# alpc91/SGRL

Measured on AMD Instinct MI355X. Metric: env-steps/sec (whole node) + SET-actor fwd us/step, 3d_walker mix @8192 envs/GPU, higher is better.
Workload: dtype f64 (dynamics) / f32 (SET actor, obs); 1 GPU; 3D_Walker++ 8 variants x 1024 envs per GPU (config 3), random U(-1,1) actions, auto-reset, SET actor forward on every step, random-init weights; envs_per_gpu=8192, obs_max_len=287, action_max_len=21, replay_gather=none (single rank)

## Files before the change

### include/sgrl_set.h

```cpp
#ifndef SGRL_SET_H
#define SGRL_SET_H

#include <stdint.h>

#ifdef __cplusplus
extern "C" {
#endif

typedef struct sgrl_set sgrl_set;

enum {
  SGRL_SET_EMB0 = 0, SGRL_SET_EMB1, SGRL_SET_EMB2, SGRL_SET_REL_W, SGRL_SET_REL_B, SGRL_SET_FNORM_W, SGRL_SET_FNORM_B,
  SGRL_SET_GENC, SGRL_SET_ENC_W, SGRL_SET_ENC_B, SGRL_SET_GGPROJ, SGRL_SET_L1G_W, SGRL_SET_L1G_B, SGRL_SET_L2G_W,
  SGRL_SET_L2G_B, SGRL_SET_L1NG_W, SGRL_SET_L1NG_B, SGRL_SET_L2NG_W, SGRL_SET_L2NG_B, SGRL_SET_DECG, SGRL_SET_L1M_W,
  SGRL_SET_L1M_B, SGRL_SET_L2M_W, SGRL_SET_L2M_B, SGRL_SET_GPROJ,
  SGRL_SET_NGLOBAL
};
enum {
  SGRL_SET_A_GPROJ = 0, SGRL_SET_A_LG1_W, SGRL_SET_A_LG1_B, SGRL_SET_A_LG2_W, SGRL_SET_A_LG2_B, SGRL_SET_QKV_W,
  SGRL_SET_QKV_B, SGRL_SET_VG_W, SGRL_SET_NGOUT_W, SGRL_SET_NGOUT_B, SGRL_SET_GOUT_W, SGRL_SET_F_GPROJ2,
  SGRL_SET_F_GPROJ3, SGRL_SET_F_LG1_W, SGRL_SET_F_LG1_B, SGRL_SET_F_LG2_W, SGRL_SET_F_LG2_B, SGRL_SET_L3_W,
  SGRL_SET_L3_B, SGRL_SET_L4_W, SGRL_SET_L4_B, SGRL_SET_L5_W, SGRL_SET_L1_W, SGRL_SET_L1_B, SGRL_SET_L2_W,
  SGRL_SET_L2_B, SGRL_SET_N1_W, SGRL_SET_N1_B, SGRL_SET_N2_W, SGRL_SET_N2_B, SGRL_SET_A_GD,
  SGRL_SET_NLAYER
// ... 13 lines not shown
  const void* src0;
  const void* src1;
  int32_t n;
  int32_t kind;
  int32_t a, b;
  float scale;
  int32_t lda, ldb;
  int32_t reserved;
} sgrl_pack_seg;
#define SGRL_SET_NSITES 7
#define SGRL_SET_NEXTRA 2
int sgrl_set_bind_params(sgrl_set* s, const sgrl_pack_seg* segs, int n_segs, const int64_t* offsets, int n_offsets,
                         int64_t total_floats);

int sgrl_set_hold_weights(sgrl_set* s, int hold);

int sgrl_set_graph(sgrl_set* s, int n_morph, const int32_t* morph_L, const int32_t* morph_count, const int32_t* trav,
                   const float* rel);
#define SGRL_SET_GRAPH_CACHE 128

int sgrl_set_forward(sgrl_set* s, const float* obs, int obs_ld, float* act, int act_ld, float max_action, void* stream);

int sgrl_set_forward_q(sgrl_set* s, const float* obs, int obs_ld, const float* action, int action_ld, float* q, int q_ld,
                       void* stream);

int sgrl_set_num_nodes(const sgrl_set* s);
int64_t sgrl_set_workspace_bytes(const sgrl_set* s);
int64_t sgrl_set_generation(const sgrl_set* s);
int sgrl_set_time_forward(sgrl_set* s, const float* obs, int obs_ld, float* act, int act_ld, float max_action,
                          int reps, void* stream, float* ms_out);
int sgrl_set_peek(sgrl_set* s, int which, float* host, int64_t n_floats);
int sgrl_set_debug_stop_after(sgrl_set* s, int stage);
int sgrl_set_debug_small_nodes(sgrl_set* s, int nodes);
int sgrl_set_last_split(const sgrl_set* s);
#define SGRL_SET_FORM_F16X3 2
#define SGRL_SET_FORM_BF16X6 3
int sgrl_set_gemm_form(sgrl_set* s, int form);
int sgrl_set_debug_product(sgrl_set* s, int kind, int form, const float* A, int lda, const float* W, int ldw, const float* bias,
                           float* C, int ldc, int M, int N, int K, const float* rowdiv, const float* aux_in, float* aux_out,
                           void* stream);
int sgrl_set_debug_chain(sgrl_set* s, int kind, const float* A, int lda, int K, const float* Wp, const float* W1, const float* b1, int hid,
                         const float* W2, const float* b2, float* C, int ldc, int M, const float* rowdiv, const float* ln, float* zc,
                         float* z2, float* fn, void* stream);
long long sgrl_set_debug_redos(int reset);
const char* sgrl_set_last_error(void);

#ifdef __cplusplus
}
#endif
#endif
```

### sgrl_amd/csrc/set_actor.hip

```cpp
#include <hip/hip_runtime.h>

#include <algorithm>
#include <cmath>
#include <cstdint>
#include <cstdlib>
#include <cstring>
#include <string>
#include <type_traits>
#include <vector>

#include "../../include/sgrl.h"
#include "../../include/sgrl_set.h"
#include "../../include/sgrl_train.h"
#include "gemm_f32.h"
#include "chain_f16.h"
#include "stream_pick.h"

namespace {

thread_local std::string g_set_err;
int sfail(int code, const std::string& msg) { g_set_err = msg; return code; }
#define SHIP_TRY(expr)                                                                     \
  do {                                                                                     \
    hipError_t _e = (expr);                                                                \
// ... 156 lines not shown
      }
      case SGRL_PACK_SUBMAT: {
        const int r = i / sg.b, c = i % sg.b;
        v = s0[(size_t)r * sg.lda + c];
        break;
      }
      default: break;
    }
    w[sg.dst + i] = v;
  }
}

__global__ void k_relbias(const float* rel, const float* Wr, const float* br, float* relb, const int32_t* m_off,
                          const int32_t* m_L, int n_morph) {
  const int k = blockIdx.x;
  if (k >= n_morph) return;
  const int L = m_L[k], off = m_off[k];
  for (int i = threadIdx.x; i < 2 * L * L; i += blockDim.x) {
    const int h = i / (L * L), ij = i % (L * L);
    const float* r = rel + (size_t)(off / 2) * 3 + ij * 3;
    relb[off + i] = Wr[h * 3] * r[0] + Wr[h * 3 + 1] * r[1] + Wr[h * 3 + 2] * r[2] + br[h];
  }
}

struct EnvTab {
  const int32_t* env_off;
  const int32_t* env_L;
  const int32_t* env_relb;
};
__global__ __launch_bounds__(256) void k_attention(const float* __restrict__ qkv, const float* __restrict__ U,
                                                   const float* __restrict__ gdir, const float* relb, EnvTab et,
                                                   int use_bias, const float* __restrict__ b_ng, const float* __restrict__ GD,
                                                   float* delta_dbg, float* g1, float* ng, int ng_ld,
                                                   const float* __restrict__ ln_w, const float* __restrict__ ln_b) {
  constexpr int LMAX = 14;
  __shared__ float sc[2 * LMAX * LMAX];
  __shared__ float gd[2 * LMAX * 3 * 2];
  __shared__ float dl[LMAX][128];
  const int e = blockIdx.x, t = threadIdx.x;
  const int n0 = et.env_off[e], L = et.env_L[e];
  {
    const int sub = t & 7;
    for (int idx = t >> 3; idx < 2 * L * L; idx += 32) {
      const int h = idx / (L * L), i = (idx / L) % L, j = idx % L;
      const float4* q = reinterpret_cast<const float4*>(qkv + (size_t)(n0 + i) * 768 + h * 128);
      const float4* k = reinterpret_cast<const float4*>(qkv + (size_t)(n0 + j) * 768 + 256 + h * 128);
      float s = 0.f;
#pragma unroll
      for (int u = 0; u < 4; u++) {
        const float4 a = q[sub + 8 * u], b = k[sub + 8 * u];
        s += a.x * b.x + a.y * b.y + a.z * b.z + a.w * b.w;
      }
      s += __shfl_xor(s, 1, 64); s += __shfl_xor(s, 2, 64); s += __shfl_xor(s, 4, 64);
      if (sub == 0) sc[idx] = use_bias ? s + relb[et.env_relb[e] + idx] : s;
    }
  }
  __syncthreads();
  if (t < 2 * L) {
    float* row = sc + t * L;
    float mx = row[0];
    for (int j = 1; j < L; j++) mx = fmaxf(mx, row[j]);
    float sum = 0.f;
    for (int j = 0; j < L; j++) { row[j] = expf(row[j] - mx); sum += row[j]; }
    for (int j = 0; j < L; j++) row[j] = row[j] / sum;
  }
  __syncthreads();
  for (int idx = t; idx < 2 * L * 6; idx += 256) {
    const int h = idx / (L * 6), i = (idx / 6) % L, se = idx % 6;
// ... 63 lines not shown
      for (int i = 0; i < LT; i++)
        if (i0 + i < L) {
          float4 o = out[i];
          const float px = __shfl_xor(o.x, 32, 64), py = __shfl_xor(o.y, 32, 64), pz = __shfl_xor(o.z, 32, 64), pw = __shfl_xor(o.w, 32, 64);
          o = h == 0 ? make_float4(o.x + px, o.y + py, o.z + pz, o.w + pw) : make_float4(px + o.x, py + o.y, pz + o.z, pw + o.w);
          if ((i & 1) == h) {
            if (quantity != 0) {
              *reinterpret_cast<float4*>(g1 + ((size_t)(n0 + i0 + i) * 3 + (quantity - 1)) * 128 + c4) = o;
            } else {
              o.x += bb.x; o.y += bb.y; o.z += bb.z; o.w += bb.w;
              *reinterpret_cast<float4*>(&dl[i0 + i][c4]) = o;
              if (delta_dbg) *reinterpret_cast<float4*>(delta_dbg + (size_t)(n0 + i0 + i) * 128 + c4) = o;
            }
          }
        }
    };
    for (int i0 = 0; i0 < L; i0 += 4) body(std::integral_constant<int, 4>{}, i0);
  }
  __syncthreads();
  const int lane = t & 63;
  const float w0 = ln_w[lane], w1 = ln_w[64 + lane], b0 = ln_b[lane], b1 = ln_b[64 + lane];
  for (int i = t >> 6; i < L; i += 4) {
    float* row = ng + (size_t)(n0 + i) * ng_ld;
    const float v0 = row[lane] + dl[i][lane], v1 = row[64 + lane] + dl[i][64 + lane];
    const float mu = wave_sum_f32(v0 + v1) * (1.f / 128.f);
    const float d0 = v0 - mu, d1 = v1 - mu;
    const float var = wave_sum_f32(d0 * d0 + d1 * d1) * (1.f / 128.f);
    const float inv = 1.0f / sqrtf(var + 1e-5f);
    row[lane] = d0 * inv * w0 + b0;
    row[64 + lane] = d1 * inv * w1 + b1;
  }
}

__global__ __launch_bounds__(256) void k_add_ln(const float* x, int ldx, const float* delta, int ldd, const float* w,
                                                const float* b, float* out1, int ld1, float* out2, int ld2, int N) {
  const int row = blockIdx.x * 4 + (threadIdx.x >> 6), lane = threadIdx.x & 63;
  if (row >= N) return;
  float v0 = x[(size_t)row * ldx + lane], v1 = x[(size_t)row * ldx + 64 + lane];
  if (delta) { v0 += delta[(size_t)row * ldd + lane]; v1 += delta[(size_t)row * ldd + 64 + lane]; }
  const float mu = wave_sum_f32(v0 + v1) * (1.f / 128.f);
  const float d0 = v0 - mu, d1 = v1 - mu;
  const float var = wave_sum_f32(d0 * d0 + d1 * d1) * (1.f / 128.f);
  const float inv = 1.0f / sqrtf(var + 1e-5f);
  const float y0 = d0 * inv * w[lane] + b[lane], y1 = d1 * inv * w[64 + lane] + b[64 + lane];
  if (out1) { out1[(size_t)row * ld1 + lane] = y0; out1[(size_t)row * ld1 + 64 + lane] = y1; }
  if (out2) { out2[(size_t)row * ld2 + lane] = y0; out2[(size_t)row * ld2 + 64 + lane] = y1; }
}

__global__ __launch_bounds__(128) void k_equiv(const float* __restrict__ T, const float* __restrict__ W5,
                                               const float* __restrict__ g1, float* g, float* outg, int N) {
  __shared__ float Ts[8 * 96];
  const int t = threadIdx.x, n0 = blockIdx.x * 8;
  const int rows = min(8, N - n0) * 3;
  for (int o = t; o < 8 * 96; o += 128) Ts[o] = (n0 + o / 96 < N) ? T[(size_t)n0 * 96 + o] : 0.f;
  float w[32];
#pragma unroll
  for (int c = 0; c < 32; c++) w[c] = W5[t * 32 + c];
  __syncthreads();
#pragma unroll
  for (int rb = 0; rb < 24; rb += 8) {
    if (rb >= rows) break;
    float gv[8], g1v[8];
#pragma unroll
    for (int r = 0; r < 8; r++) {
      const size_t row = (size_t)n0 * 3 + (rb + r < rows ? rb + r : 0);
      gv[r] = g[row * D + t];
// ... 44 lines not shown
  if (n >= N) return;
  float vec[3];
  const float mq = m2[(size_t)n * 32 + c];
  for (int s = 0; s < 3; s++) {
    float v = z[(size_t)n * 96 + s * 32 + c] * mq;
    for (int off = 16; off > 0; off >>= 1) v += __shfl_xor(v, off, 32);
    vec[s] = v;
  }
  if (c < 3) {
    const int env = nt.node_env[n], limb = nt.node_limb[n];
    const float* o = obs + (size_t)env * obs_ld + 41 * limb + 3 * (5 + c);
    const float a = o[0] * vec[0] + o[1] * vec[1] + o[2] * vec[2];
    act[(size_t)env * act_ld + 3 * limb + c] = max_action * tanhf(a);
  }
}

__global__ __launch_bounds__(256) void k_q_head(const float* __restrict__ c, const float* __restrict__ w, const float* __restrict__ b,
                                                const float* __restrict__ fn, NodeTab nt, float* q, int q_ld, int N) {
  const int n = blockIdx.x * 4 + (threadIdx.x >> 6), lane = threadIdx.x & 63;
  if (n >= N) return;
  const float* row = c + (size_t)n * 256;
  float v = row[lane] * w[lane] + row[64 + lane] * w[64 + lane] + row[128 + lane] * w[128 + lane] + row[192 + lane] * w[192 + lane];
  v = wave_sum_f32(v);
  if (lane == 0) q[(size_t)nt.node_env[n] * q_ld + nt.node_limb[n]] = (v + b[0]) / fn[n];
}

}

struct GraphCfg {
  std::vector<int32_t> key_i;
  std::vector<float> key_f;
  int n_env = 0, N = 0, n_morph = 0, TM = 0, Lmax = 0;
  int split_env = 0, split_node = 0;
  int32_t *d_node_env = nullptr, *d_node_limb = nullptr, *d_node_mnode = nullptr, *d_trav = nullptr;
  int32_t *d_env_off = nullptr, *d_env_L = nullptr, *d_env_relb = nullptr, *d_m_off = nullptr, *d_m_L = nullptr;
  float *d_rel = nullptr, *d_relb = nullptr;
  uint64_t last_use = 0;
  void release() {
    void* ptrs[] = {d_node_env, d_node_limb, d_node_mnode, d_trav, d_env_off, d_env_L, d_env_relb, d_m_off, d_m_L, d_rel, d_relb};
    for (void* q : ptrs) if (q) (void)hipFree(q);
  }
};

struct sgrl_set {
  const float* w = nullptr;
  int64_t off[SGRL_SET_NW];
  bool have_w = false, have_graph = false;
  int n_env = 0, N = 0, n_morph = 0, TM = 0, Lmax = 0;
  int split_env = 0, split_node = 0;
  int last_split = 0;
  int32_t *d_node_env = nullptr, *d_node_limb = nullptr, *d_node_mnode = nullptr, *d_trav = nullptr;
  int32_t *d_env_off = nullptr, *d_env_L = nullptr, *d_env_relb = nullptr, *d_m_off = nullptr, *d_m_L = nullptr;
  float *d_rel = nullptr, *d_relb = nullptr;
  std::vector<GraphCfg*> cfgs;
  uint64_t use_clock = 0;
  int64_t generation = 0;
  float* ws = nullptr;
  int64_t ws_floats = 0;
  int carved_N = 0;
  float* cat_cur = nullptr;
  float *g, *cat, *cat2, *zc, *fn, *h256, *qkv, *vg, *g1, *z2, *mat, *t256, *t256b, *t128a, *t128b, *delta,
      *outg, *outng, *gdir;
  float* wstack = nullptr;
  const float* site_ptr[SGRL_SET_NSITES];
  bool hold = false, packed_ok = false;
  int packed_form = 0;
  hipEvent_t ev_pack = nullptr;
  const float* l2mf_w = nullptr;
  const float* l2mf_b = nullptr;
  unsigned short* d_tri = nullptr;
  bool stack_dirty = true;
  bool stack_critic = false;
  int stop_after = -1;
  int small_nodes = -1;
  int gemm_form = 0;
  sgrl_gemm::EncMat* d_enc = nullptr;
  int n_enc = 0, enc_rows = 0;
  float* wsc = nullptr;
  std::vector<std::pair<int64_t, int>> enc_index;
  bool live = false;
  float* wflat = nullptr;
  unsigned* wwords = nullptr;
  int64_t wflat_floats = 0;
// ... 37 lines not shown
  int best = 0, best_rank = -1;
  int64_t best_dist = 0;
  for (size_t e = 1; e < env_off.size(); e++) {
    const int n = env_off[e];
    const int64_t dist = std::abs(2 * (int64_t)n - N);
    const int rank = 2 * dist > N / 16 ? 0 : (n % 128 == 0 ? 3 : n % 64 == 0 ? 2 : 1);
    if (best_rank < 0 || rank > best_rank || (rank == best_rank && dist < best_dist)) { best = (int)e; best_rank = rank; best_dist = dist; }
  }
  *env_out = best;
  *node_out = best ? env_off[best] : 0;
}

int use_cfg(sgrl_set* s, GraphCfg* c) {
  const int64_t N = c->N;
  const int64_t need = ws_floats_for(N);
  if (need > s->ws_floats) {
    if (s->ws) { (void)hipFree(s->ws); s->generation++; }
    s->ws = nullptr; s->ws_floats = 0; s->carved_N = 0;
    if (hipMalloc(&s->ws, sizeof(float) * need) != hipSuccess) return sfail(SGRL_ERR_HIP, "device allocation failed (SET workspace)");
    s->ws_floats = need;
  }
  if (s->carved_N != c->N) {
    float* p = s->ws;
    auto take = [&](int64_t n) { float* r = p; p += (n + 31) & ~int64_t(31); return r; };
    s->g = take(384 * N); s->cat = take(256 * N); s->cat2 = take(256 * N); s->zc = take(96 * N); s->fn = take(N);
    s->h256 = take(256 * N); s->qkv = take(768 * N); s->vg = take(768 * N);
    s->g1 = take(384 * N); s->z2 = take(96 * N); s->mat = take(96 * N); s->t256 = take(256 * N); s->t256b = take(256 * N); s->t128a = take(128 * N);
    s->t128b = take(128 * N); s->delta = take(128 * N); s->outg = take(3 * OGLD * N); s->outng = take(160 * N); s->gdir = take(6 * N);
    if (p - s->ws > s->ws_floats) return sfail(SGRL_ERR_LIMIT, "workspace carve-up overflow");
    s->carved_N = c->N;
  }
  s->n_env = c->n_env; s->N = c->N; s->n_morph = c->n_morph; s->TM = c->TM; s->Lmax = c->Lmax;
  s->split_env = c->split_env; s->split_node = c->split_node;
  s->d_node_env = c->d_node_env; s->d_node_limb = c->d_node_limb; s->d_node_mnode = c->d_node_mnode; s->d_trav = c->d_trav;
  s->d_env_off = c->d_env_off; s->d_env_L = c->d_env_L; s->d_env_relb = c->d_env_relb; s->d_m_off = c->d_m_off; s->d_m_L = c->d_m_L;
  s->d_rel = c->d_rel; s->d_relb = c->d_relb;
  c->last_use = ++s->use_clock;
  s->have_graph = true;
  return SGRL_OK;
}

bool gemm_use_split() {
  static const bool v = [] { const char* e = getenv("SGRL_SET_GEMM"); return !(e && e[0] == 'f'); }();
  return v;
}
struct GemmCtx {
  int form = SGRL_SET_FORM_F16X3;
  const float* w_base = nullptr; const unsigned* w_words = nullptr;
  const float* wsc = nullptr;
  const std::vector<std::pair<int64_t, int>>* enc_index = nullptr;
};
int gemm_default_form() {
  static const int v = [] { const char* e = getenv("SGRL_SET_GEMM"); return (e && e[0] == 'b') ? SGRL_SET_FORM_BF16X6 : SGRL_SET_FORM_F16X3; }();
  return v;
}
const float* wsc_of(const GemmCtx& gx, const float* W) {
  if (!gx.enc_index) return nullptr;
  const int64_t off = W - gx.w_base;
  for (const auto& e : *gx.enc_index) if (e.first == off) return gx.wsc + e.second;
  return nullptr;
}
GemmArgs with_words(const GemmCtx& gx, const GemmArgs& a) {
  GemmArgs b = a;
  b.W = reinterpret_cast<const float*>(gx.w_words + (a.W - gx.w_base));
  b.wscale = wsc_of(gx, a.W);
  return b;
// ... 304 lines not shown
    if (encode) join(whole);
    if (s->live && !reuse && !capturing) {
      s->packed_ok = s->hold;
      s->packed_form = want_words ? SGRL_SET_FORM_F16X3 : SGRL_SET_FORM_BF16X6;
      if (s->hold) (void)hipEventRecord(s->ev_pack, st);
    }
    s->cat_cur = s->cat;
    if (!s->live && (s->stack_dirty || s->stack_critic != critic)) {
      s->stack_critic = critic;
      auto sw = [&](int site) { return s->wstack + (size_t)site * 64 * 128; };
      for (int l = 0; l < SGRL_SET_LAYERS; l++) {
        hipLaunchKernelGGL(k_stack_proj, dim3(32), dim3(256), 0, st, s->WL(l, SGRL_SET_A_GPROJ), (const float*)nullptr, D, D, sw(2 * l));
        hipLaunchKernelGGL(k_stack_proj, dim3(32), dim3(256), 0, st, s->WL(l, SGRL_SET_F_GPROJ2), s->WL(l, SGRL_SET_F_GPROJ3), D, D, sw(2 * l + 1));
      }
      hipLaunchKernelGGL(k_stack_proj, dim3(36), dim3(256), 0, st, s->W(SGRL_SET_GGPROJ), critic ? (const float*)nullptr : s->W(SGRL_SET_GPROJ), 136, OGLD, sw(6));
      s->stack_dirty = false;
    }
  }
  int attn_site(const Part& p, int l) const {
    fork(p);
    int rc = gemm(p.sd, p.g, D, s->WL(l, SGRL_SET_VG_W), D, nullptr, p.vg, 256, 3 * p.M, 256, D);
    if (rc == SGRL_OK)
      rc = site(p, p.g, D, D, 2 * l, nullptr, s->WL(l, SGRL_SET_A_LG1_W), s->WL(l, SGRL_SET_A_LG1_B), 256, p.h256, s->WL(l, SGRL_SET_A_LG2_W),
                s->WL(l, SGRL_SET_A_LG2_B), p.catc);
    if (rc != SGRL_OK) return rc;
    if (l == 0 && p.ev_site0) (void)hipEventRecord(p.ev_site0, p.st);
    rc = gemm(p.st, p.catc, 256, s->WL(l, SGRL_SET_QKV_W), 256, s->WL(l, SGRL_SET_QKV_B), p.qkv, 768, p.M, 768, 256, EPI_ROWDIV, p.fn);
    if (rc != SGRL_OK) return rc;
    join(p);
    return SGRL_OK;
  }
  int attention(const Part& p, int l) const {
    const EnvTab etp{et.env_off + p.e0, et.env_L + p.e0, et.env_relb + p.e0};
    hipLaunchKernelGGL(k_attention, dim3(p.ne), dim3(256), 0, p.st, s->qkv, s->vg, s->gdir, s->d_relb, etp, l == 0 ? 1 : 0,
                       s->WL(l, SGRL_SET_NGOUT_B), s->WL(l, SGRL_SET_A_GD), s->stop_after == 2 * l ? s->delta : (float*)nullptr,
                       s->g1, p.catc - 256 * (size_t)p.r0 + 128, 256, s->WL(l, SGRL_SET_N1_W), s->WL(l, SGRL_SET_N1_B));
    return s->stop_after == 2 * l ? kStop : SGRL_OK;
  }
  int ffn_site(const Part& p, int l) const {
    return site(p, p.g1, D, D, 2 * l + 1, p.z2, s->WL(l, SGRL_SET_F_LG1_W), s->WL(l, SGRL_SET_F_LG1_B), 256, p.h256, s->WL(l, SGRL_SET_F_LG2_W),
                s->WL(l, SGRL_SET_F_LG2_B), p.catc);
  }
  int norm2_unfused(const Part& p, int l) const {
    float* const ng = p.catc + 128;
    if (!one_stream) {
      (void)hipEventRecord(s->ev_l3, p.st);
      (void)hipStreamWaitEvent(p.sd, s->ev_l3, 0);
    }
    if (!small)
      return launch_gemm_ln(gx, p.sd, p.t256b, 256, s->WL(l, SGRL_SET_L2_W), 256, s->WL(l, SGRL_SET_L2_B), p.M, 256, p.fn, ng, 256,
                            s->WL(l, SGRL_SET_N2_W), s->WL(l, SGRL_SET_N2_B));
    const int rc = small_gemm(p.st, p.t256b, 256, s->WL(l, SGRL_SET_L2_W), 256, s->WL(l, SGRL_SET_L2_B), p.delta, 128, p.M, 128, 256, EPI_ROWDIV, p.fn);
    if (rc != SGRL_OK) return rc;
    hipLaunchKernelGGL(k_add_ln, dim3((p.M + 3) / 4), dim3(256), 0, p.st, ng, 256, p.delta, 128, s->WL(l, SGRL_SET_N2_W),
                       s->WL(l, SGRL_SET_N2_B), (float*)nullptr, 0, ng, 256, p.M);
    return SGRL_OK;
  }
  int ffn_tail(Part& p, int l) const {
    fork(p);
    int rc;
    if (chain) {
      rc = launch_chain_ln(gx, p.sd, p.catc, 256, 256, s->WL(l, SGRL_SET_L1_W), s->WL(l, SGRL_SET_L1_B), s->WL(l, SGRL_SET_L2_W), s->WL(l, SGRL_SET_L2_B),
                           p.fn, p.catc + 128, 256, s->WL(l, SGRL_SET_N2_W), s->WL(l, SGRL_SET_N2_B), p.M, p.cato + 128);
    } else {
      rc = gemm(p.sd, p.catc, 256, s->WL(l, SGRL_SET_L1_W), 256, s->WL(l, SGRL_SET_L1_B), p.t256b, 256, p.M, 256, 256, EPI_RELU);
    }
    if (rc == SGRL_OK) rc = gemm(p.st, p.catc, 256, s->WL(l, SGRL_SET_L3_W), 256, s->WL(l, SGRL_SET_L3_B), p.t256, 256, p.M, 256, 256, EPI_RELU);
    if (rc == SGRL_OK && !chain) rc = norm2_unfused(p, l);
    if (rc == SGRL_OK) rc = equiv_gemm(p, p.t256, s->WL(l, SGRL_SET_L4_W), s->WL(l, SGRL_SET_L4_B));
// ... 347 lines not shown
          travT[(size_t)q * TM + m_node0[k] + i] = v;
        }
      tp += 3 * (size_t)L;
    }
  }
  for (int k = 0; k < n_morph; k++) {
    for (int c = 0; c < morph_count[k]; c++) {
      env_off.push_back(node);
      env_L.push_back(morph_L[k]);
      env_relb.push_back(m_off[k]);
      for (int i = 0; i < morph_L[k]; i++) {
        node_env.push_back(env);
        node_limb.push_back(i);
        node_mnode.push_back(m_node0[k] + i);
        node++;
      }
      env++;
    }
  }
  if (node == 0) return sfail(SGRL_ERR_ARG, "no environments");
  if ((int)s->cfgs.size() >= SGRL_SET_GRAPH_CACHE) {
    size_t lru = 0;
    for (size_t i = 1; i < s->cfgs.size(); i++) if (s->cfgs[i]->last_use < s->cfgs[lru]->last_use) lru = i;
    s->cfgs[lru]->release();
    s->generation++;
    delete s->cfgs[lru];
    s->cfgs.erase(s->cfgs.begin() + lru);
  }
  GraphCfg* c = new GraphCfg();
  c->key_i = std::move(key_i);
  c->key_f.assign(rel, rel + nrel);
  c->n_env = env; c->N = node; c->n_morph = n_morph; c->TM = TM; c->Lmax = Lmax;
  pick_split(env_off, node, &c->split_env, &c->split_node);
  bool ok = upload(&c->d_node_env, node_env) == 0 && upload(&c->d_node_limb, node_limb) == 0 &&
            upload(&c->d_node_mnode, node_mnode) == 0 && upload(&c->d_trav, travT) == 0 &&
            upload(&c->d_env_off, env_off) == 0 && upload(&c->d_env_L, env_L) == 0 && upload(&c->d_env_relb, env_relb) == 0 &&
            upload(&c->d_m_off, m_off) == 0 && upload(&c->d_m_L, m_L) == 0 && upload(&c->d_rel, c->key_f) == 0;
  if (ok) ok = hipMalloc(&c->d_relb, sizeof(float) * relb_off) == hipSuccess;
  if (!ok) { c->release(); delete c; return sfail(SGRL_ERR_HIP, "device allocation failed in sgrl_set_graph"); }
  s->cfgs.push_back(c);
  return use_cfg(s, c);
}

int sgrl_set_forward(sgrl_set* s, const float* obs, int obs_ld, float* act, int act_ld, float max_action, void* stream) {
  if (!s || !obs || !act) return sfail(SGRL_ERR_ARG, "sgrl_set_forward: null argument");
  if (!s->have_w || !s->have_graph) return sfail(SGRL_ERR_ARG, "sgrl_set_forward: weights or graph not set");
  if (obs_ld < 41 * s->Lmax || act_ld < 3 * s->Lmax)
    return sfail(SGRL_ERR_ARG, "sgrl_set_forward: obs_ld < 41 * Lmax or act_ld < 3 * Lmax (rows too narrow for the largest morphology)");
  return run_forward(s, obs, obs_ld, act, act_ld, max_action, (hipStream_t)stream);
}

int sgrl_set_forward_q(sgrl_set* s, const float* obs, int obs_ld, const float* action, int action_ld, float* q, int q_ld,
                       void* stream) {
  if (!s || !obs || !action || !q) return sfail(SGRL_ERR_ARG, "sgrl_set_forward_q: null argument");
  if (!s->have_w || !s->have_graph) return sfail(SGRL_ERR_ARG, "sgrl_set_forward_q: weights or graph not set");
  if (obs_ld < 41 * s->Lmax || action_ld < 3 * s->Lmax || q_ld < s->Lmax)
    return sfail(SGRL_ERR_ARG, "sgrl_set_forward_q: obs_ld < 41 * Lmax, action_ld < 3 * Lmax or q_ld < Lmax");
  return run_forward(s, obs, obs_ld, q, q_ld, 0.f, (hipStream_t)stream, true, action, action_ld);
}

int sgrl_set_time_forward(sgrl_set* s, const float* obs, int obs_ld, float* act, int act_ld, float max_action,
                          int reps, void* stream, float* ms_out) {
  if (!s || !obs || !act || !ms_out || reps <= 0) return sfail(SGRL_ERR_ARG, "sgrl_set_time_forward: bad argument");
  if (!s->have_w || !s->have_graph) return sfail(SGRL_ERR_ARG, "weights or graph not set");
  if (obs_ld < 41 * s->Lmax || act_ld < 3 * s->Lmax) return sfail(SGRL_ERR_ARG, "sgrl_set_time_forward: rows too narrow for the largest morphology");
  hipEvent_t t0, t1;
// ... 15 lines not shown
}

int sgrl_set_hold_weights(sgrl_set* s, int hold) {
  if (!s) return sfail(SGRL_ERR_ARG, "sgrl_set_hold_weights: null handle");
  s->hold = hold != 0;
  s->packed_ok = false;
  return SGRL_OK;
}

int sgrl_set_num_nodes(const sgrl_set* s) { return s ? s->N : SGRL_ERR_ARG; }
int64_t sgrl_set_workspace_bytes(const sgrl_set* s) { return s ? s->ws_floats * 4 : -1; }
int64_t sgrl_set_generation(const sgrl_set* s) { return s ? s->generation : -1; }
int sgrl_set_last_split(const sgrl_set* s) { return s ? s->last_split : SGRL_ERR_ARG; }

int sgrl_set_peek(sgrl_set* s, int which, float* host, int64_t n_floats) {
  if (!s || !host || !s->have_graph) return sfail(SGRL_ERR_ARG, "sgrl_set_peek: bad argument");
  const float* src[] = {s->g, s->cat_cur ? s->cat_cur : s->cat, s->zc, s->fn, s->qkv, nullptr, nullptr, s->mat, s->g1, s->delta, s->outng};
  const int64_t per[] = {384, 256, 96, 1, 768, 0, 0, 96, 384, 128, 160};
  if (which < 0 || which > 10 || !src[which] || n_floats > per[which] * s->N) return sfail(SGRL_ERR_ARG, "sgrl_set_peek: bad buffer or size");
  SHIP_TRY(hipDeviceSynchronize());
  SHIP_TRY(hipMemcpy(host, src[which], sizeof(float) * n_floats, hipMemcpyDeviceToHost));
  return SGRL_OK;
}

int sgrl_set_debug_stop_after(sgrl_set* s, int stage) {
  if (!s || stage < -1 || stage >= 2 * SGRL_SET_LAYERS) return sfail(SGRL_ERR_ARG, "sgrl_set_debug_stop_after: bad argument");
  s->stop_after = stage;
  return SGRL_OK;
}

int sgrl_set_debug_small_nodes(sgrl_set* s, int nodes) {
  if (!s || nodes < -1) return sfail(SGRL_ERR_ARG, "sgrl_set_debug_small_nodes: bad argument");
  s->small_nodes = nodes;
  return SGRL_OK;
}

int sgrl_set_gemm_form(sgrl_set* s, int form) {
  if (!s || (form != 0 && form != SGRL_SET_FORM_F16X3 && form != SGRL_SET_FORM_BF16X6)) return sfail(SGRL_ERR_ARG, "sgrl_set_gemm_form: bad argument");
  if (s->gemm_form != form) s->generation++;
  s->gemm_form = form;
  return SGRL_OK;
}

namespace {
struct TempWords {
  unsigned* w = nullptr; float* sc = nullptr; sgrl_gemm::EncMat* dm = nullptr;
  ~TempWords() { if (w) (void)hipFree(w); if (sc) (void)hipFree(sc); if (dm) (void)hipFree(dm); }
  int make(hipStream_t st, const float* W, int rows, int K, int group = 1) {
    const sgrl_gemm::EncMat m{0, rows, K, 0, group};
    if (hipMalloc(&w, sizeof(unsigned) * (size_t)rows * K) != hipSuccess || hipMalloc(&sc, sizeof(float) * rows) != hipSuccess ||
        hipMalloc(&dm, sizeof(m)) != hipSuccess || hipMemcpy(dm, &m, sizeof(m), hipMemcpyHostToDevice) != hipSuccess)
      return sfail(SGRL_ERR_HIP, "debug product: allocation failed");
    hipLaunchKernelGGL(sgrl_gemm::k_encode_rows, dim3((rows + 3) / 4), dim3(256), 0, st, W, w, sc, dm, 1, rows);
    return SGRL_OK;
  }
};
}

int sgrl_set_debug_product(sgrl_set* s, int kind, int form, const float* A, int lda, const float* W, int ldw, const float* bias,
                           float* C, int ldc, int M, int N, int K, const float* rowdiv, const float* aux_in, float* aux_out,
                           void* stream) {
  if (!s || !A || !W || !C || M <= 0 || N <= 0 || K <= 0) return sfail(SGRL_ERR_ARG, "sgrl_set_debug_product: bad argument");
  hipStream_t st = (hipStream_t)stream;
  if (!GemmKernels<0>::raise_lds_limits() || !GemmKernels<EPI_RELU>::raise_lds_limits() || !GemmKernels<EPI_ROWDIV>::raise_lds_limits())
    return sfail(SGRL_ERR_HIP, "cannot raise the dynamic LDS limit of the tile kernels");
  TempWords tw;
// ... 111 lines not shown
```

### sgrl_amd/set_hip.py

```python
import ctypes

import numpy as np
import torch

from . import _lib

NGLOBAL, NLAYER, LAYERS = 25, 31, 3
NW = NGLOBAL + LAYERS * NLAYER


def _bind(L):
    if getattr(L, "_set_bound", False):
        return
    vp = ctypes.c_void_p
    L.sgrl_set_create.argtypes = [ctypes.POINTER(vp)]
    L.sgrl_set_destroy.argtypes = [vp]
    L.sgrl_set_destroy.restype = None
    L.sgrl_set_weights.argtypes = [vp, vp, vp, ctypes.c_int]
    L.sgrl_set_bind_params.argtypes = [vp, vp, ctypes.c_int, vp, ctypes.c_int, ctypes.c_int64]
    L.sgrl_set_graph.argtypes = [vp, ctypes.c_int, vp, vp, vp, vp]
    L.sgrl_set_forward.argtypes = [vp, vp, ctypes.c_int, vp, ctypes.c_int, ctypes.c_float, vp]
    L.sgrl_set_forward_q.argtypes = [vp, vp, ctypes.c_int, vp, ctypes.c_int, vp, ctypes.c_int, vp]
    L.sgrl_set_time_forward.argtypes = [vp, vp, ctypes.c_int, vp, ctypes.c_int, ctypes.c_float, ctypes.c_int, vp,
                                        ctypes.POINTER(ctypes.c_float)]
    L.sgrl_set_num_nodes.argtypes = [vp]
    L.sgrl_set_workspace_bytes.argtypes = [vp]
    L.sgrl_set_workspace_bytes.restype = ctypes.c_int64
    L.sgrl_set_generation.argtypes = [vp]
    L.sgrl_set_generation.restype = ctypes.c_int64
    L.sgrl_set_peek.argtypes = [vp, ctypes.c_int, vp, ctypes.c_int64]
    L.sgrl_set_debug_stop_after.argtypes = [vp, ctypes.c_int]
    L.sgrl_set_debug_small_nodes.argtypes = [vp, ctypes.c_int]
    L.sgrl_set_last_split.argtypes = [vp]
    L.sgrl_set_gemm_form.argtypes = [vp, ctypes.c_int]
    L.sgrl_set_last_error.restype = ctypes.c_char_p
    L.sgrl_set_hold_weights.argtypes = [vp, ctypes.c_int]
    L.sgrl_set_debug_redos.argtypes = [ctypes.c_int]
    L.sgrl_set_debug_redos.restype = ctypes.c_longlong
    ci = ctypes.c_int
    L.sgrl_set_debug_product.argtypes = [vp, ci, ci, vp, ci, vp, ci, vp, vp, ci, ci, ci, ci, vp, vp, vp, vp]
    L.sgrl_set_debug_chain.argtypes = [vp, ci, vp, ci, ci, vp, vp, vp, ci, vp, vp, vp, ci, ci, vp, vp, vp, vp, vp, vp]
    L._set_bound = True


def _check(L, rc, what):
    if rc != 0:
        raise _lib.SgrlError("%s failed (%d): %s" % (what, rc, L.sgrl_set_last_error().decode()))


GRAM_K = 576


def gram_order():
    a, b, ok = [], [], []
    for A in range(8):
        for B in range(A + 1):
            for i in range(4):
                for j in range(4):
                    a.append(4 * A + i); b.append(4 * B + j); ok.append(4 * A + i >= 4 * B + j)
    return torch.tensor(a), torch.tensor(b), torch.tensor(ok)


def fold_gram_weight(w):
    out_f = w.shape[0]
    w3 = w.reshape(out_f, 32, 32)
# ... 303 lines not shown
        assert obs.shape[1] >= 41 * self.max_limbs and action.shape[1] >= 3 * self.max_limbs
        self.sync_weights()
        q_ld = q_ld or self.max_limbs
        assert q_ld >= self.max_limbs
        if out is None:
            out = torch.empty((self.n_env, q_ld), dtype=torch.float32, device=self.device)
        assert out.is_contiguous() and out.shape == (self.n_env, q_ld)
        _check(self.L, self.L.sgrl_set_forward_q(self.h, ctypes.c_void_p(obs.data_ptr()), self._ld(obs),
                                                 ctypes.c_void_p(action.data_ptr()), self._ld(action),
                                                 ctypes.c_void_p(out.data_ptr()), int(q_ld), self._stream()),
               "sgrl_set_forward_q")
        return out

    def time_forward(self, obs, out, reps):
        self.sync_weights()
        ms = ctypes.c_float(0)
        _check(self.L, self.L.sgrl_set_time_forward(self.h, ctypes.c_void_p(obs.data_ptr()), self._ld(obs),
                                                    ctypes.c_void_p(out.data_ptr()), self._ld(out),
                                                    ctypes.c_float(float(self.policy.max_action)), int(reps),
                                                    self._stream(), ctypes.byref(ms)), "sgrl_set_time_forward")
        return float(ms.value)

    def forward_single(self, state, graph):
        B = state.shape[0]
        self.configure([graph], [B])
        return self.forward_batch(state.contiguous().float(), act_ld=3 * len(graph["parents"]))

    def debug_stop_after(self, stage):
        _check(self.L, self.L.sgrl_set_debug_stop_after(self.h, int(stage)), "sgrl_set_debug_stop_after")

    def debug_small_nodes(self, nodes):
        _check(self.L, self.L.sgrl_set_debug_small_nodes(self.h, int(nodes)), "sgrl_set_debug_small_nodes")

    def last_split(self):
        return int(self.L.sgrl_set_last_split(self.h))

    FORM_F16X3, FORM_BF16X6 = 2, 3

    def gemm_form(self, form):
        _check(self.L, self.L.sgrl_set_gemm_form(self.h, int(form)), "sgrl_set_gemm_form")

    def hold_weights(self, hold=True):
        self.sync_weights()
        _check(self.L, self.L.sgrl_set_hold_weights(self.h, 1 if hold else 0), "sgrl_set_hold_weights")

    def scale_redos(self, reset=True):
        return int(self.L.sgrl_set_debug_redos(1 if reset else 0))

    def peek(self, which, per_node):
        out = np.zeros((self.num_nodes, per_node), dtype=np.float32)
        _check(self.L, self.L.sgrl_set_peek(self.h, which, ctypes.c_void_p(out.ctypes.data), out.size), "sgrl_set_peek")
        return out


class HipSetCritic(object):

    def __init__(self, critic_module, device=None):
        self.q1 = HipSetActor(critic_module, device=device, net=critic_module.critic1, critic=True)
        self.q2 = HipSetActor(critic_module, device=device, net=critic_module.critic2, critic=True)

    def configure(self, graphs, counts):
        self.q1.configure(graphs, counts)
        self.q2.configure(graphs, counts)

    def forward_batch(self, obs, action, q_ld=None, which=(1, 2)):
        out = []
# ... 11 lines not shown
```

Baseline: 1.927 million env-steps/s.

## Add limb-count-specialized attention kernel for small morphologies

Adds a templated attention kernel specialized per limb count (2..8) that keeps V rows and outputs in registers, splits the 256-thread block into four quantity groups (value plus three U directions), and uses wave-level barriers instead of block barriers between softmax, gdir mixing and the weighted sum. Environments in that range go to the new kernel. The general kernel now early-exits for them and is launched only when the graph also has morphologies outside the range. The aim is to cut per-environment attention overhead from runtime-L loops and shared-memory traffic. In exchange it adds template instantiations, higher register pressure under a 5-wave launch bound, and a possible second launch for mixed graphs.

```diff
diff --git a/include/sgrl_set.h b/include/sgrl_set.h
--- a/include/sgrl_set.h
+++ b/include/sgrl_set.h
@@ -69,6 +69,7 @@
 int sgrl_set_peek(sgrl_set* s, int which, float* host, int64_t n_floats);
 int sgrl_set_debug_stop_after(sgrl_set* s, int stage);
 int sgrl_set_debug_small_nodes(sgrl_set* s, int nodes);
+int sgrl_set_debug_attention(sgrl_set* s, int form);
 int sgrl_set_last_split(const sgrl_set* s);
 #define SGRL_SET_FORM_F16X3 2
 #define SGRL_SET_FORM_BF16X6 3
diff --git a/sgrl_amd/csrc/set_actor.hip b/sgrl_amd/csrc/set_actor.hip
--- a/sgrl_amd/csrc/set_actor.hip
+++ b/sgrl_amd/csrc/set_actor.hip
@@ -212,8 +212,10 @@
                                                    const float* __restrict__ gdir, const float* relb, EnvTab et,
                                                    int use_bias, const float* __restrict__ b_ng, const float* __restrict__ GD,
                                                    float* delta_dbg, float* g1, float* ng, int ng_ld,
-                                                   const float* __restrict__ ln_w, const float* __restrict__ ln_b) {
+                                                   const float* __restrict__ ln_w, const float* __restrict__ ln_b,
+                                                   int skip_lo, int skip_hi) {
   constexpr int LMAX = 14;
+  if (const int Le = et.env_L[blockIdx.x]; Le >= skip_lo && Le <= skip_hi) return;
   __shared__ float sc[2 * LMAX * LMAX];
   __shared__ float gd[2 * LMAX * 3 * 2];
   __shared__ float dl[LMAX][128];
@@ -343,6 +345,197 @@
   }
 }
 
+constexpr int kAttnLimbsLo = 2, kAttnLimbsHi = 8;
+constexpr int kAttnLimbsWaves = 5;
+template <int LC, bool DBG>
+__device__ __forceinline__ void attention_limbs(const float* __restrict__ qkv, const float* __restrict__ U, const float* __restrict__ gdir,
+                                                const float* relb, int relb_off, int use_bias, const float* __restrict__ b_ng,
+                                                const float* __restrict__ GD, float* delta_dbg, float* g1, float* ng, int ng_ld,
+                                                const float* __restrict__ ln_w, const float* __restrict__ ln_b, const int n0,
+                                                float* sc, float* wts_all, float* gd_all, float (*dl)[128]) {
+  constexpr int NS = 2 * LC * LC;
+  constexpr int NIT = (NS + 31) / 32;
+  constexpr int NB0 = LC < 4 ? LC : 4;
+  constexpr int NB1 = LC - NB0;
+  const int t = threadIdx.x, quantity = t >> 6, ln = t & 63, h = ln >> 5, c4 = (ln & 31) * 4;
+  float* const wts = wts_all + quantity * 128;
+  float* const gds = gd_all + quantity * 32;
+  const float* vbase = quantity == 0 ? qkv + (size_t)n0 * 768 + 512 + h * 128 + c4
+                                     : U + ((size_t)n0 * 3 + (quantity - 1)) * 256 + h * 128 + c4;
+  const int gh = ln / (2 * LC), gi = (ln >> 1) % LC, ge = ln & 1;
+  const bool gd_lane = quantity != 0 && ln < 4 * LC;
+  {
+    const int sub = t & 7;
+#pragma unroll 1
+    for (int k = 0; k < NIT; k++) {
+      const int idx = (t >> 3) + 32 * k;
+      if (idx < NS) {
+        const float rb = use_bias ? relb[relb_off + idx] : 0.f;
+        const int hh = idx / (LC * LC), i = (idx / LC) % LC, j = idx % LC;
+        const float4* q = reinterpret_cast<const float4*>(qkv + (size_t)(n0 + i) * 768 + hh * 128);
+        const float4* kk = reinterpret_cast<const float4*>(qkv + (size_t)(n0 + j) * 768 + 256 + hh * 128);
+        float s = 0.f;
+#pragma unroll
+        for (int u = 0; u < 4; u++) {
+          const float4 a = q[sub + 8 * u], b = kk[sub + 8 * u];
+          s += a.x * b.x + a.y * b.y + a.z * b.z + a.w * b.w;
+        }
+        s += __shfl_xor(s, 1, 64); s += __shfl_xor(s, 2, 64); s += __shfl_xor(s, 4, 64);
+        if (sub == 0) sc[idx] = use_bias ? s + rb : s;
+      }
+    }
+  }
+  float4 v0[NB0];
+#pragma unroll
+  for (int j = 0; j < NB0; j++) v0[j] = *reinterpret_cast<const float4*>(vbase + (size_t)j * 768);
+  float4 v1[NB1 > 0 ? NB1 : 1];
+#pragma unroll
+  for (int j = 0; j < NB1; j++) v1[j] = *reinterpret_cast<const float4*>(vbase + (size_t)(NB0 + j) * 768);
+  float gdv[LC];
+#pragma unroll
+  for (int j = 0; j < LC; j++) gdv[j] = gd_lane ? gdir[(size_t)(n0 + j) * 6 + 2 * (quantity - 1) + ge] : 0.f;
+  __syncthreads();
+  if (ln < 2 * LC) {
+    float p[LC];
+#pragma unroll
+    for (int j = 0; j < LC; j++) p[j] = sc[ln * LC + j];
+    float mx = p[0];
+#pragma unroll
+    for (int j = 1; j < LC; j++) mx = fmaxf(mx, p[j]);
+    float sum = 0.f;
+#pragma unroll
+    for (int j = 0; j < LC; j++) { p[j] = expf(p[j] - mx); sum += p[j]; }
+#pragma unroll
+    for (int j = 0; j < LC; j++) wts[(ln / LC) * LC * LC + j * LC + ln % LC] = p[j] / sum;
+  }
+  __builtin_amdgcn_fence(__ATOMIC_RELEASE, "wavefront");
+  __builtin_amdgcn_wave_barrier();
+  __builtin_amdgcn_fence(__ATOMIC_ACQUIRE, "wavefront");
+  if (gd_lane) {
+    const float* w = wts + gh * LC * LC + gi;
+    float s = 0.f;
+#pragma unroll
+    for (int j = 0; j < LC; j++) s += w[j * LC] * gdv[j];
+    gds[(gh * LC + gi) * 2 + ge] = s;
+  }
+  __builtin_amdgcn_fence(__ATOMIC_RELEASE, "wavefront");
+  __builtin_amdgcn_wave_barrier();
+  __builtin_amdgcn_fence(__ATOMIC_ACQUIRE, "wavefront");
+  {
+    float4 out[LC];
+#pragma unroll
+    for (int i = 0; i < LC; i++) out[i] = make_float4(0.f, 0.f, 0.f, 0.f);
+    const float* wh = wts + h * LC * LC;
+    float4 ga = make_float4(0.f, 0.f, 0.f, 0.f), gb = ga, bb = ga;
+    if (quantity != 0) {
+      ga = *reinterpret_cast<const float4*>(GD + (h * 128 + c4) * 2);
+      gb = *reinterpret_cast<const float4*>(GD + (h * 128 + c4) * 2 + 4);
+    } else {
+      bb = *reinterpret_cast<const float4*>(b_ng + c4);
+    }
+#pragma unroll
+    for (int j = 0; j < LC; j++) {
+      const float4 v = j < NB0 ? v0[j < NB0 ? j : 0] : v1[j >= NB0 ? j - NB0 : 0];
+#pragma unroll
+      for (int i = 0; i < LC; i++) {
+        const float w = wh[j * LC + i];
+        out[i].x += w * v.x; out[i].y += w * v.y; out[i].z += w * v.z; out[i].w += w * v.w;
+      }
+    }
+    if (quantity != 0) {
+#pragma unroll
+      for (int i = 0; i < LC; i++) {
+        const float* gg = gds + (h * LC + i) * 2;
+        const float g0 = gg[0], g1v = gg[1];
+        out[i].x += ga.x * g0 + ga.y * g1v; out[i].y += ga.z * g0 + ga.w * g1v;
+        out[i].z += gb.x * g0 + gb.y * g1v; out[i].w += gb.z * g0 + gb.w * g1v;
+      }
+    }
+#pragma unroll
+    for (int i = 0; i < LC; i++) {
+      float4 o = out[i];
+      const float px = __shfl_xor(o.x, 32, 64), py = __shfl_xor(o.y, 32, 64), pz = __shfl_xor(o.z, 32, 64), pw = __shfl_xor(o.w, 32, 64);
+      o = h == 0 ? make_float4(o.x + px, o.y + py, o.z + pz, o.w + pw) : make_float4(px + o.x, py + o.y, pz + o.z, pw + o.w);
+      if ((i & 1) == h) {
+        if (quantity != 0) {
+          *reinterpret_cast<float4*>(g1 + ((size_t)(n0 + i) * 3 + (quantity - 1)) * 128 + c4) = o;
+        } else {
+          o.x += bb.x; o.y += bb.y; o.z += bb.z; o.w += bb.w;
+          *reinterpret_cast<float4*>(&dl[i][c4]) = o;
+          if constexpr (DBG) *reinterpret_cast<float4*>(delta_dbg + (size_t)(n0 + i) * 128 + c4) = o;
+        }
+      }
+    }
+  }
+  float x0[2], x1[2];
+#pragma unroll
+  for (int r = 0; r < 2; r++) {
+    const int i = quantity + 4 * r;
+    x0[r] = x1[r] = 0.f;
+    if (i < LC) {
+      const float* row = ng + (size_t)(n0 + i) * ng_ld;
+      x0[r] = row[ln];
+      x1[r] = row[64 + ln];
+    }
+  }
+  const float w0 = ln_w[ln], w1 = ln_w[64 + ln], b0 = ln_b[ln], b1 = ln_b[64 + ln];
+  __syncthreads();
+#pragma unroll
+  for (int r = 0; r < 2; r++) {
+    const int i = quantity + 4 * r;
+    if (i < LC) {
+      float* row = ng + (size_t)(n0 + i) * ng_ld;
+      const float v0n = x0[r] + dl[i][ln], v1n = x1[r] + dl[i][64 + ln];
+      const float mu = wave_sum_f32(v0n + v1n) * (1.f / 128.f);
+      const float d0 = v0n - mu, d1 = v1n - mu;
+      const float var = wave_sum_f32(d0 * d0 + d1 * d1) * (1.f / 128.f);
+      const float inv = 1.0f / sqrtf(var + 1e-5f);
+      row[ln] = d0 * inv * w0 + b0;
+      row[64 + ln] = d1 * inv * w1 + b1;
+    }
+  }
+}
+
+#ifdef SGRL_ATTN_RESOURCE_PROBE
+template <int LC>
+__global__ __launch_bounds__(256, kAttnLimbsWaves) void k_attention_probe(const float* qkv, const float* U, const float* gdir, const float* relb, const float* b_ng,
+                                                         const float* GD, float* g1, float* ng, const float* ln_w, const float* ln_b, int n0) {
+  __shared__ float sc[2 * LC * LC], wts[4 * 128], gd[4 * 32], dl[LC][128];
+  attention_limbs<LC, false>(qkv, U, gdir, relb, 0, n0 & 1, b_ng, GD, nullptr, g1, ng, 256, ln_w, ln_b, n0, sc, wts, gd, dl);
+}
+template __global__ void k_attention_probe<2>(const float*, const float*, const float*, const float*, const float*, const float*, float*, float*, const float*, const float*, int);
+template __global__ void k_attention_probe<3>(const float*, const float*, const float*, const float*, const float*, const float*, float*, float*, const float*, const float*, int);
+template __global__ void k_attention_probe<4>(const float*, const float*, const float*, const float*, const float*, const float*, float*, float*, const float*, const float*, int);
+template __global__ void k_attention_probe<5>(const float*, const float*, const float*, const float*, const float*, const float*, float*, float*, const float*, const float*, int);
+template __global__ void k_attention_probe<6>(const float*, const float*, const float*, const float*, const float*, const float*, float*, float*, const float*, const float*, int);
+template __global__ void k_attention_probe<7>(const float*, const float*, const float*, const float*, const float*, const float*, float*, float*, const float*, const float*, int);
+template __global__ void k_attention_probe<8>(const float*, const float*, const float*, const float*, const float*, const float*, float*, float*, const float*, const float*, int);
+#endif
+
+template <bool DBG>
+__global__ __launch_bounds__(256, kAttnLimbsWaves) void k_attention_limbs(const float* __restrict__ qkv, const float* __restrict__ U,
+                                                         const float* __restrict__ gdir, const float* relb, EnvTab et, int use_bias,
+                                                         const float* __restrict__ b_ng, const float* __restrict__ GD,
+                                                         float* delta_dbg, float* g1, float* ng, int ng_ld,
+                                                         const float* __restrict__ ln_w, const float* __restrict__ ln_b) {
+  __shared__ float sc[2 * kAttnLimbsHi * kAttnLimbsHi];
+  __shared__ float wts[4 * 2 * kAttnLimbsHi * kAttnLimbsHi];
+  __shared__ float gd[4 * 2 * kAttnLimbsHi * 2];
+  __shared__ float dl[kAttnLimbsHi][128];
+  const int e = blockIdx.x, L = et.env_L[e];
+  if (L < kAttnLimbsLo || L > kAttnLimbsHi) return;
+  const int n0 = et.env_off[e], ro = use_bias ? et.env_relb[e] : 0;
+#define SGRL_ATTN_CASE(LC)                                                                                                       \
+  case LC:                                                                                                                       \
+    attention_limbs<LC, DBG>(qkv, U, gdir, relb, ro, use_bias, b_ng, GD, delta_dbg, g1, ng, ng_ld, ln_w, ln_b, n0, sc, wts, gd, dl); \
+    break;
+  switch (L) {
+    SGRL_ATTN_CASE(2) SGRL_ATTN_CASE(3) SGRL_ATTN_CASE(4) SGRL_ATTN_CASE(5) SGRL_ATTN_CASE(6) SGRL_ATTN_CASE(7) SGRL_ATTN_CASE(8)
+    default: break;
+  }
+#undef SGRL_ATTN_CASE
+}
+
 __global__ __launch_bounds__(256) void k_add_ln(const float* x, int ldx, const float* delta, int ldd, const float* w,
                                                 const float* b, float* out1, int ld1, float* out2, int ld2, int N) {
   const int row = blockIdx.x * 4 + (threadIdx.x >> 6), lane = threadIdx.x & 63;
@@ -453,6 +646,7 @@
   std::vector<float> key_f;
   int n_env = 0, N = 0, n_morph = 0, TM = 0, Lmax = 0;
   int split_env = 0, split_node = 0;
+  bool attn_limbs = false, attn_general = false;
   int32_t *d_node_env = nullptr, *d_node_limb = nullptr, *d_node_mnode = nullptr, *d_trav = nullptr;
   int32_t *d_env_off = nullptr, *d_env_L = nullptr, *d_env_relb = nullptr, *d_m_off = nullptr, *d_m_L = nullptr;
   float *d_rel = nullptr, *d_relb = nullptr;
@@ -470,6 +664,8 @@
   int n_env = 0, N = 0, n_morph = 0, TM = 0, Lmax = 0;
   int split_env = 0, split_node = 0;
   int last_split = 0;
+  bool attn_limbs = false, attn_general = false;
+  int attn_form = 1;
   int32_t *d_node_env = nullptr, *d_node_limb = nullptr, *d_node_mnode = nullptr, *d_trav = nullptr;
   int32_t *d_env_off = nullptr, *d_env_L = nullptr, *d_env_relb = nullptr, *d_m_off = nullptr, *d_m_L = nullptr;
   float *d_rel = nullptr, *d_relb = nullptr;
@@ -573,6 +769,7 @@
   }
   s->n_env = c->n_env; s->N = c->N; s->n_morph = c->n_morph; s->TM = c->TM; s->Lmax = c->Lmax;
   s->split_env = c->split_env; s->split_node = c->split_node;
+  s->attn_limbs = c->attn_limbs; s->attn_general = c->attn_general;
   s->d_node_env = c->d_node_env; s->d_node_limb = c->d_node_limb; s->d_node_mnode = c->d_node_mnode; s->d_trav = c->d_trav;
   s->d_env_off = c->d_env_off; s->d_env_L = c->d_env_L; s->d_env_relb = c->d_env_relb; s->d_m_off = c->d_m_off; s->d_m_L = c->d_m_L;
   s->d_rel = c->d_rel; s->d_relb = c->d_relb;
@@ -943,9 +1140,17 @@
   }
   int attention(const Part& p, int l) const {
     const EnvTab etp{et.env_off + p.e0, et.env_L + p.e0, et.env_relb + p.e0};
-    hipLaunchKernelGGL(k_attention, dim3(p.ne), dim3(256), 0, p.st, s->qkv, s->vg, s->gdir, s->d_relb, etp, l == 0 ? 1 : 0,
-                       s->WL(l, SGRL_SET_NGOUT_B), s->WL(l, SGRL_SET_A_GD), s->stop_after == 2 * l ? s->delta : (float*)nullptr,
-                       s->g1, p.catc - 256 * (size_t)p.r0 + 128, 256, s->WL(l, SGRL_SET_N1_W), s->WL(l, SGRL_SET_N1_B));
+    float* const dbg = s->stop_after == 2 * l ? s->delta : (float*)nullptr;
+    float* const ng = p.catc - 256 * (size_t)p.r0 + 128;
+    const bool limbs = s->attn_form != 0 && s->attn_limbs;
+    if (limbs)
+      hipLaunchKernelGGL(dbg ? k_attention_limbs<true> : k_attention_limbs<false>, dim3(p.ne), dim3(256), 0, p.st, s->qkv, s->vg, s->gdir,
+                         s->d_relb, etp, l == 0 ? 1 : 0, s->WL(l, SGRL_SET_NGOUT_B), s->WL(l, SGRL_SET_A_GD), dbg, s->g1, ng, 256,
+                         s->WL(l, SGRL_SET_N1_W), s->WL(l, SGRL_SET_N1_B));
+    if (!limbs || s->attn_general)
+      hipLaunchKernelGGL(k_attention, dim3(p.ne), dim3(256), 0, p.st, s->qkv, s->vg, s->gdir, s->d_relb, etp, l == 0 ? 1 : 0,
+                         s->WL(l, SGRL_SET_NGOUT_B), s->WL(l, SGRL_SET_A_GD), dbg, s->g1, ng, 256, s->WL(l, SGRL_SET_N1_W),
+                         s->WL(l, SGRL_SET_N1_B), limbs ? kAttnLimbsLo : 1, limbs ? kAttnLimbsHi : 0);
     return s->stop_after == 2 * l ? kStop : SGRL_OK;
   }
   int ffn_site(const Part& p, int l) const {
@@ -1359,6 +1564,8 @@
   c->key_f.assign(rel, rel + nrel);
   c->n_env = env; c->N = node; c->n_morph = n_morph; c->TM = TM; c->Lmax = Lmax;
   pick_split(env_off, node, &c->split_env, &c->split_node);
+  for (int k = 0; k < n_morph; k++)
+    if (morph_count[k] > 0) (morph_L[k] >= kAttnLimbsLo && morph_L[k] <= kAttnLimbsHi ? c->attn_limbs : c->attn_general) = true;
   bool ok = upload(&c->d_node_env, node_env) == 0 && upload(&c->d_node_limb, node_limb) == 0 &&
             upload(&c->d_node_mnode, node_mnode) == 0 && upload(&c->d_trav, travT) == 0 &&
             upload(&c->d_env_off, env_off) == 0 && upload(&c->d_env_L, env_L) == 0 && upload(&c->d_env_relb, env_relb) == 0 &&
@@ -1440,6 +1647,13 @@
 int sgrl_set_debug_small_nodes(sgrl_set* s, int nodes) {
   if (!s || nodes < -1) return sfail(SGRL_ERR_ARG, "sgrl_set_debug_small_nodes: bad argument");
   s->small_nodes = nodes;
+  return SGRL_OK;
+}
+
+int sgrl_set_debug_attention(sgrl_set* s, int form) {
+  if (!s || (form != 0 && form != 1)) return sfail(SGRL_ERR_ARG, "sgrl_set_debug_attention: bad argument");
+  if (s->attn_form != form) s->generation++;
+  s->attn_form = form;
   return SGRL_OK;
 }
 
diff --git a/sgrl_amd/set_hip.py b/sgrl_amd/set_hip.py
--- a/sgrl_amd/set_hip.py
+++ b/sgrl_amd/set_hip.py
@@ -31,6 +31,7 @@
     L.sgrl_set_peek.argtypes = [vp, ctypes.c_int, vp, ctypes.c_int64]
     L.sgrl_set_debug_stop_after.argtypes = [vp, ctypes.c_int]
     L.sgrl_set_debug_small_nodes.argtypes = [vp, ctypes.c_int]
+    L.sgrl_set_debug_attention.argtypes = [vp, ctypes.c_int]
     L.sgrl_set_last_split.argtypes = [vp]
     L.sgrl_set_gemm_form.argtypes = [vp, ctypes.c_int]
     L.sgrl_set_last_error.restype = ctypes.c_char_p
@@ -400,6 +401,9 @@
     def debug_small_nodes(self, nodes):
         _check(self.L, self.L.sgrl_set_debug_small_nodes(self.h, int(nodes)), "sgrl_set_debug_small_nodes")
 
+    def debug_attention(self, form):
+        _check(self.L, self.L.sgrl_set_debug_attention(self.h, int(form)), "sgrl_set_debug_attention")
+
     def last_split(self):
         return int(self.L.sgrl_set_last_split(self.h))
 
```

After: 1.955 million env-steps/s (median of 6 runs). 1.01x the previous value.
